# jdalcorso/radar-sounder-crw

Measured on AMD Instinct MI355X. Metric: radargram columns/sec (CRW fwd+bwd), higher is better.
Workload: dtype f32 (conv2-5 multiply on the bf16 matrix cores with hi/lo operand pairs, fp32 accumulate: fp32-grade; everything else fp32); 1 GPU; one synthetic 512x4096 radargram per GPU per step = 8 items [T=32,N=63,16x16] (patch 16x16, overlap (8, 0)), tau=0.01, CNN encoder, fwd+bwd+all-reduce+Adam; parallelism=dp1 (independent sequences), chain=fp32 MFMA 16x16x4, prefix form, encoder_convs=bf16x3

## Files before the change

radar-sounder-crw_amd/csrc/encoder_conv.hip:

```cpp
#include "crw_common.h"
#include <type_traits>
#include <cstdlib>

namespace crw {
namespace {

constexpr int IMG_W = 10, PAD_W = 12, NPIX = 100, NPAD = 144, MT = 7;

typedef __bf16 bf8 __attribute__((ext_vector_type(8)));
typedef short s4v __attribute__((ext_vector_type(4)));
typedef short s8v __attribute__((ext_vector_type(8)));
typedef __attribute__((address_space(3))) char *lds_cp;

__device__ inline uint16_t f2bf(float x) { return __builtin_bit_cast(uint16_t, (__bf16)x); }
__device__ inline float bf2f(uint16_t h) { return __builtin_bit_cast(float, (uint32_t)h << 16); }

template <int C>
constexpr int row_stride() { return C * 2 + 16; }
template <int C>
constexpr int plane_bytes() { return NPAD * row_stride<C>(); }
template <int C>
__device__ inline int px_off(int pp, int chunk) { return pp * row_stride<C>() + 16 * chunk; }
template <int C>
constexpr int crs() { return C * 2 + 32; }
// ... 481 lines not shown
  constexpr int NCO = WG_NCO, NTH = NW * 64;
  constexpr int NPL = (SPLIT == 3) ? 2 : 1;
  constexpr int XS = row_stride<NCI>(), XPL = (XTAIL + NPAD) * XS;
  constexpr int YS = row_stride<NCO>(), YPL = YROWS_ALL * YS;
  constexpr int NT = NCI / 16;
  constexpr int WCI = NT < 4 ? NT : 4, WCO = NW / WCI;
  constexpr int NCOW = NCO / 16 / WCO;
  static_assert(NT == WCI && COUT % NCO == 0 && CIN % NCI == 0, "tiling");
  constexpr int NGRP_CI = CIN / NCI;
  extern __shared__ __attribute__((aligned(16))) char lds[];
  char *xs = lds, *ys = lds + NPL * XPL;

  constexpr int NGRP = NGRP_CI * (COUT / NCO);
  const int wg_slice = a.xcd_map ? ((int)blockIdx.x / 8 / NGRP) * 8 + (int)blockIdx.x % 8 : (int)blockIdx.x / NGRP;
  const int wg_grp = a.xcd_map ? ((int)blockIdx.x / 8) % NGRP : (int)blockIdx.x % NGRP;
  const int grp_ci = wg_grp % NGRP_CI, grp_co = wg_grp / NGRP_CI;
  const int ci_base = grp_ci * NCI, co_base = grp_co * NCO;
  const int tid = threadIdx.x, lane = tid & 63, wave = tid >> 6, g = lane >> 4;
  const int wci = wave % WCI, wco = wave / WCI;
  const int co0w = wco * NCOW * 16;

  f32x4 acc[9][NCOW];
#pragma unroll
  for (int t = 0; t < 9; ++t)
#pragma unroll
    for (int j = 0; j < NCOW; ++j) acc[t][j] = f32x4{0.f, 0.f, 0.f, 0.f};
  f32x4 accb[NCOW];
#pragma unroll
  for (int j = 0; j < NCOW; ++j) accb[j] = f32x4{0.f, 0.f, 0.f, 0.f};
  const bool bias_wave = grp_ci == 0 && __builtin_amdgcn_readfirstlane(wci) == 0;

  const int p_begin = wg_slice * a.patches_per_block;
  const int p_end = min(a.P, p_begin + a.patches_per_block);
  const uint32_t xs_a = (uint32_t)(uintptr_t)(lds_cp)xs, ys_a = (uint32_t)(uintptr_t)(lds_cp)ys;

  for (int pl = 0; pl < NPL; ++pl) {
    zero_halo<NCI, NTH, XS>(xs + pl * XPL + XTAIL * XS, tid);
    for (int c = tid; c < XTAIL * XS / 16; c += NTH) *reinterpret_cast<uint4 *>(xs + pl * XPL + 16 * c) = uint4{0, 0, 0, 0};
    for (int c = tid; c < (1 + TAILPIX) * YS / 16; c += NTH) *reinterpret_cast<uint4 *>(ys + pl * YPL + NPIX * YS + 16 * c) = uint4{0, 0, 0, 0};
  }

  constexpr int XCH = NCI / 8, XTOT = NPIX * XCH, XIT = (XTOT + NTH - 1) / NTH;
  constexpr int YCH = NCO / 8, YTOT = NPIX * YCH, YIT = (YTOT + NTH - 1) / NTH;
  constexpr int TXC = XTAIL * XCH, TYC = TAILPIX * YCH, TTOT = NPL * (TXC + TYC), TIT = (TTOT + NTH - 1) / NTH;
#ifdef CRW_CONV_STAMPS
  long long ph_[4] = {0, 0, 0, 0}, prev_ = (long long)__builtin_amdgcn_s_memtime();
#define WG_STAMP(k) { const long long n_ = (long long)__builtin_amdgcn_s_memtime(); ph_[k] += n_ - prev_; prev_ = n_; }
#else
#define WG_STAMP(k)
#endif

  auto tail_src_dst = [&](int c, int &src, int &dst) {
    const int pl = c / (TXC + TYC), r = c % (TXC + TYC);
    if (r < TXC) {
      const int s = r / XCH, ch = r % XCH;
      dst = pl * XPL + s * XS + 16 * ch;
      src = pl * XPL + (XTAIL + 9 * PAD_W + s) * XS + 16 * ch;
    } else {
      const int q = r - TXC, j = q / YCH, ch = q % YCH;
      dst = NPL * XPL + pl * YPL + (YROWS + j) * YS + 16 * ch;
      src = NPL * XPL + pl * YPL + (NPIX - TAILPIX + j) * YS + 16 * ch;
    }
  };

  const int t16 = lane & 15, q4 = t16 >> 2, pq = t16 & 3;
  const uint32_t lane_col = 8 * (pq & 1) + 16 * (pq >> 1);
  auto row_addr = [&](int v, int carry, bool flush, uint32_t &ya, uint32_t &xa) {
    const int i = v - carry;
    int yrow = NPIX, xpix = XTAIL;
    if (v < carry) {
      const int t = NPIX - carry + v;
      yrow = YROWS + (t - (NPIX - TAILPIX));
      xpix = t - 90;
    } else if (!flush && i < NPIX) {
      yrow = i;
      xpix = XTAIL + (i / IMG_W) * PAD_W + (i % IMG_W);
    }
    ya = ys_a + yrow * YS + lane_col + 2 * co0w;
    xa = xs_a + xpix * XS + lane_col + 32 * wci;
  };
  auto kstep = [&](int ks, int carry, bool flush) {
    uint32_t ya_lo, ya_hi, xa_lo, xa_hi;
    row_addr(32 * ks + 4 * g + q4, carry, flush, ya_lo, xa_lo);
    row_addr(32 * ks + 4 * g + q4 + 16, carry, flush, ya_hi, xa_hi);
    bf8 ah[NCOW], al[NCOW];
    static_for<NCOW>([&](auto JC) {
      constexpr int j = decltype(JC)::value;
      ah[j] = tr_frag<32 * j>(ya_lo, ya_hi);
      if (SPLIT == 3) al[j] = tr_frag<YPL + 32 * j>(ya_lo, ya_hi);
    });
    bf8 bh[2], bl[2];
    auto read_b = [&](auto TC) {
      constexpr int tap = decltype(TC)::value;
      constexpr int XO = ((tap / 3) * PAD_W + (tap % 3)) * XS;
      bh[tap & 1] = tr_frag<XO>(xa_lo, xa_hi);
      if (SPLIT == 3) bl[tap & 1] = tr_frag<XPL + XO>(xa_lo, xa_hi);
    };
    read_b(std::integral_constant<int, 0>{});
    static_for<9>([&](auto TC) {
      constexpr int tap = decltype(TC)::value;
      if constexpr (tap < 8) {
        read_b(std::integral_constant<int, tap + 1>{});
        if (SPLIT == 3) asm volatile("s_waitcnt lgkmcnt(4)" ::: "memory");
        else asm volatile("s_waitcnt lgkmcnt(2)" ::: "memory");
      } else {
        asm volatile("s_waitcnt lgkmcnt(0)" ::: "memory");
      }
      __builtin_amdgcn_sched_barrier(0);
      if constexpr (tap == 0) {
        if (bias_wave) {
          const s8v o = {0x3f80, 0x3f80, 0x3f80, 0x3f80, 0x3f80, 0x3f80, 0x3f80, 0x3f80};
          const bf8 ones = __builtin_bit_cast(bf8, o);
#pragma unroll
          for (int j = 0; j < NCOW; ++j) {
            if (SPLIT == 3) accb[j] = __builtin_amdgcn_mfma_f32_16x16x32_bf16(al[j], ones, accb[j], 0, 0, 0);
            accb[j] = __builtin_amdgcn_mfma_f32_16x16x32_bf16(ah[j], ones, accb[j], 0, 0, 0);
          }
        }
      }
#pragma unroll
      for (int j = 0; j < NCOW; ++j) {
        if (SPLIT == 3) {
          acc[tap][j] = __builtin_amdgcn_mfma_f32_16x16x32_bf16(al[j], bh[tap & 1], acc[tap][j], 0, 0, 0);
          acc[tap][j] = __builtin_amdgcn_mfma_f32_16x16x32_bf16(ah[j], bl[tap & 1], acc[tap][j], 0, 0, 0);
        }
        acc[tap][j] = __builtin_amdgcn_mfma_f32_16x16x32_bf16(ah[j], bh[tap & 1], acc[tap][j], 0, 0, 0);
      }
    });
  };

  int carry = 0;
  uint4 tv[TIT];
#pragma unroll
  for (int i = 0; i < TIT; ++i) tv[i] = uint4{0, 0, 0, 0};
  if constexpr (MAP) {
    const int ntile = a.tiles_x * a.tiles_y;
    constexpr int WTOT = NPAD * XCH, WIT = (WTOT + NTH - 1) / NTH;
    for (int u = p_begin; u < p_end; ++u) {
      const int pq = u / ntile, tile = u % ntile;
      const int ty0 = (tile / a.tiles_x) * IMG_W, tx0 = (tile % a.tiles_x) * IMG_W;
      __syncthreads();
      for (int pl = 0; pl < NPL; ++pl) {
        uint4 xv[WIT];
        const uint16_t *src = (pl ? a.xl : a.xh) + ci_base;
#pragma unroll
        for (int i = 0; i < WIT; ++i) {
          const int c = min(tid + i * NTH, WTOT - 1), wp = c / XCH, ch = c % XCH;
          const int my = ty0 + wp / PAD_W - 1, mx = tx0 + wp % PAD_W - 1;
          const bool ok = my >= 0 && my < a.mh && mx >= 0 && mx < a.mw;
          const long off = (((long)pq * a.mh + min(max(my, 0), a.mh - 1)) * a.mw + min(max(mx, 0), a.mw - 1)) * CIN + 8 * ch;
          xv[i] = *reinterpret_cast<const uint4 *>(src + off);
          if (!ok) xv[i] = uint4{0, 0, 0, 0};
        }
#pragma unroll
        for (int i = 0; i < WIT; ++i) {
          const int c = tid + i * NTH;
          if (WTOT % NTH == 0 || c < WTOT) *reinterpret_cast<uint4 *>(xs + pl * XPL + (XTAIL + c / XCH) * XS + 16 * (c % XCH)) = xv[i];
        }
        uint4 yv[YIT];
        const uint16_t *ysrc = (pl ? a.dyl : a.dyh) + co_base;
#pragma unroll
        for (int i = 0; i < YIT; ++i) {
          const int c = min(tid + i * NTH, YTOT - 1), pix = c / YCH, ch = c % YCH;
          const int oy = ty0 + pix / IMG_W, ox = tx0 + pix % IMG_W;
          const bool ok = oy < a.mh && ox < a.mw;
          const long off = (((long)pq * a.mh + min(oy, a.mh - 1)) * a.mw + min(ox, a.mw - 1)) * COUT + 8 * ch;
          yv[i] = *reinterpret_cast<const uint4 *>(ysrc + off);
          if (!ok) yv[i] = uint4{0, 0, 0, 0};
        }
#pragma unroll
        for (int i = 0; i < YIT; ++i) {
          const int c = tid + i * NTH;
          if (YTOT % NTH == 0 || c < YTOT) *reinterpret_cast<uint4 *>(ys + pl * YPL + (c / YCH) * YS + 16 * (c % YCH)) = yv[i];
        }
      }
      __syncthreads();
#pragma unroll 1
      for (int ks = 0; ks < 4; ++ks) kstep(ks, 0, false);
    }
  }
  for (int p = MAP ? p_end : p_begin; p < p_end; ++p) {
    __syncthreads();
    WG_STAMP(3)
    {
#pragma unroll
      for (int i = 0; i < TIT; ++i) {
        const int c = tid + i * NTH;
        if (TTOT % NTH == 0 || c < TTOT) {
          int src, dst;
          tail_src_dst(c, src, dst);
          *reinterpret_cast<uint4 *>(xs + dst) = tv[i];
        }
      }
      uint4 xv[NPL][XIT], yv[NPL][YIT];
#pragma unroll
      for (int pl = 0; pl < NPL; ++pl) {
        const uint16_t *src = (pl ? a.xl : a.xh) + (long)p * NPIX * CIN + ci_base;
#pragma unroll
        for (int i = 0; i < XIT; ++i) {
          const int c = min(tid + i * NTH, XTOT - 1);
          xv[pl][i] = *reinterpret_cast<const uint4 *>(src + (long)(c / XCH) * CIN + 8 * (c % XCH));
        }
      }
#pragma unroll
      for (int pl = 0; pl < NPL; ++pl) {
        const uint16_t *src = ((pl && !a.dgap) ? a.dyl : a.dyh) + (long)p * NPIX * COUT + co_base;
#pragma unroll
        for (int i = 0; i < YIT; ++i) {
          const int c = min(tid + i * NTH, YTOT - 1);
          yv[pl][i] = *reinterpret_cast<const uint4 *>(src + (long)(c / YCH) * COUT + 8 * (c % YCH));
        }
      }
#pragma unroll
      for (int pl = 0; pl < NPL; ++pl)
#pragma unroll
        for (int i = 0; i < XIT; ++i) {
          const int c = tid + i * NTH;
          if (XTOT % NTH == 0 || c < XTOT)
            *reinterpret_cast<uint4 *>(xs + pl * XPL + (XTAIL + interior_pp(c / XCH)) * XS + 16 * (c % XCH)) = xv[pl][i];
        }
      if (a.dgap) {
        static_assert(NTH % YCH == 0, "a thread keeps its channel chunk");
        const int ch = tid % YCH;
        uint32_t gh[4], gl[4];
        gap_split8(a.dgap + (long)p * COUT + co_base + 8 * ch, gh, gl);
#pragma unroll
        for (int i = 0; i < YIT; ++i) {
          const int c = tid + i * NTH;
          if (YTOT % NTH == 0 || c < YTOT) {
            uint4 oh, ol;
            gap_mask8(yv[0][i], gh, gl, oh, ol);
            const int off = (c / YCH) * YS + 16 * ch;
            *reinterpret_cast<uint4 *>(ys + off) = oh;
            if (SPLIT == 3) *reinterpret_cast<uint4 *>(ys + YPL + off) = ol;
          }
        }
      } else {
#pragma unroll
        for (int pl = 0; pl < NPL; ++pl)
#pragma unroll
          for (int i = 0; i < YIT; ++i) {
            const int c = tid + i * NTH;
            if (YTOT % NTH == 0 || c < YTOT) *reinterpret_cast<uint4 *>(ys + pl * YPL + (c / YCH) * YS + 16 * (c % YCH)) = yv[pl][i];
          }
      }
    }
    __syncthreads();
    WG_STAMP(0)
    WG_STAMP(1)
#ifdef CRW_CONV_STAMPS
    if (a.stamps && tid == 0 && p - p_begin < 60)
      a.stamps[(long)blockIdx.x * 64 + 4 + (p - p_begin)] = (long long)__builtin_amdgcn_s_memtime();
#endif
    const int nks = carry == 8 ? 4 : 3;
#pragma unroll 1
    for (int ks = 0; ks < nks; ++ks) kstep(ks, carry, false);
    carry = carry == 8 ? 0 : carry + 4;
#pragma unroll
    for (int i = 0; i < TIT; ++i) {
      const int c = min(tid + i * NTH, TTOT - 1);
      int src, dst;
      tail_src_dst(c, src, dst);
      tv[i] = *reinterpret_cast<const uint4 *>(xs + src);
    }
    WG_STAMP(2)
  }
  if (carry > 0) {
    __syncthreads();
#pragma unroll
    for (int i = 0; i < TIT; ++i) {
      const int c = tid + i * NTH;
      if (TTOT % NTH == 0 || c < TTOT) {
        int src, dst;
        tail_src_dst(c, src, dst);
        *reinterpret_cast<uint4 *>(xs + dst) = tv[i];
      }
    }
    __syncthreads();
    kstep(0, carry, true);
  }
#ifdef CRW_CONV_STAMPS
  if (a.stamps && tid == 0)
    for (int k = 0; k < 4; ++k) a.stamps[(long)blockIdx.x * 64 + k] = ph_[k];
#endif

  float *dwp = a.dw_part + (long)wg_slice * COUT * CIN * 9;
#pragma unroll
  for (int tap = 0; tap < 9; ++tap)
#pragma unroll
    for (int j = 0; j < NCOW; ++j)
#pragma unroll
      for (int r = 0; r < 4; ++r) {
        const int co = co_base + co0w + 16 * j + 4 * g + r, ci = ci_base + 16 * wci + (lane & 15);
        dwp[((long)tap * COUT + co) * CIN + ci] = acc[tap][j][r];
      }
  if (bias_wave && (lane & 15) == 0) {
#pragma unroll
    for (int j = 0; j < NCOW; ++j)
#pragma unroll
      for (int r = 0; r < 4; ++r) a.db_part[(long)wg_slice * COUT + co_base + co0w + 16 * j + 4 * g + r] = accb[j][r];
  }
}

constexpr int W2_NCO = 128, W2_NCI = 64, W2_NW = 8, W2_KROWS = 32;
template <int C>
constexpr int w2_stride() { return 2 * C + 32; }

template <int SPLIT, int CIN, int COUT, int DIAG = 0>
__global__ __launch_bounds__(W2_NW * 64, 2) void conv3x3_wgrad2_kernel(WgradArgs a) {
  constexpr int NCO = W2_NCO, NCI = W2_NCI, NTH = W2_NW * 64, NPL = (SPLIT == 3) ? 2 : 1;
  constexpr int XS = w2_stride<NCI>(), XPL = NPAD * XS, XSLOT = NPL * XPL;
  constexpr int YS = w2_stride<NCO>(), YPL = W2_KROWS * YS, YSLOT = NPL * YPL;
  constexpr int NCOW = 4, WCI = 4;
  static_assert(COUT == NCO && CIN % NCI == 0, "tiling");
  constexpr int NGRP = CIN / NCI;
  extern __shared__ __attribute__((aligned(16))) char lds[];
  char *xs = lds, *ys = lds + 2 * XSLOT;
  char *gs = ys + 2 * YSLOT;

  const int wg_slice = a.xcd_map ? ((int)blockIdx.x / 8 / NGRP) * 8 + (int)blockIdx.x % 8 : (int)blockIdx.x / NGRP;
  const int grp_ci = a.xcd_map ? ((int)blockIdx.x / 8) % NGRP : (int)blockIdx.x % NGRP;
  const int ci_base = grp_ci * NCI;
  const int tid = threadIdx.x, lane = tid & 63, wave = tid >> 6, g = lane >> 4;
  const int wci = wave % WCI, wco = wave / WCI;
  const int wci_s = __builtin_amdgcn_readfirstlane(wci);
  const int co0w = wco * NCOW * 16;

  const int p_begin = wg_slice * a.patches_per_block;
  const int np = min(a.P, p_begin + a.patches_per_block) - p_begin;
  const int npx = np * NPIX;
  const int NK = (npx + W2_KROWS - 1) / W2_KROWS;

  f32x4 acc[9][NCOW];
#pragma unroll
  for (int t = 0; t < 9; ++t)
#pragma unroll
    for (int j = 0; j < NCOW; ++j) acc[t][j] = f32x4{0.f, 0.f, 0.f, 0.f};
  f32x4 accb = f32x4{0.f, 0.f, 0.f, 0.f};
  const bool bias_wg = grp_ci == 0;

  for (int c = tid; c < 2 * XSLOT / 16; c += NTH) *reinterpret_cast<uint4 *>(xs + 16 * c) = uint4{0, 0, 0, 0};

  const int yrow = tid >> 4, ych = tid & 15;
  constexpr int XCH = NCI / 8, XTOT = NPIX * XCH;
  typedef uint32_t u4v __attribute__((ext_vector_type(4)));
  const long dy_off = (long)p_begin * NPIX * COUT, x_off = (long)p_begin * NPIX * CIN + ci_base;
  const __amdgpu_buffer_rsrc_t dyh_rs = __builtin_amdgcn_make_buffer_rsrc((void *)(a.dyh + dy_off), 0, npx * COUT * 2, 0x00020000);
  const __amdgpu_buffer_rsrc_t dyl_rs = __builtin_amdgcn_make_buffer_rsrc(
      (void *)((SPLIT == 3 && !a.dgap ? a.dyl : a.dyh) + dy_off), 0, npx * COUT * 2, 0x00020000);
  const __amdgpu_buffer_rsrc_t xh_rs = __builtin_amdgcn_make_buffer_rsrc((void *)(a.xh + x_off), 0, (npx * CIN - ci_base) * 2, 0x00020000);
  const __amdgpu_buffer_rsrc_t xl_rs = __builtin_amdgcn_make_buffer_rsrc((void *)((SPLIT == 3 ? a.xl : a.xh) + x_off), 0,
                                                                          (npx * CIN - ci_base) * 2, 0x00020000);
  const int y_voff = (yrow * COUT + 8 * ych) * 2;
  int x_voff[2];
#pragma unroll
  for (int i = 0; i < 2; ++i) {
    const int c = min(tid + i * NTH, XTOT - 1);
    x_voff[i] = ((c / XCH) * CIN + 8 * (c % XCH)) * 2;
  }
  uint4 sy[NPL], sx[2];
  auto load_dy = [&](int n) {
    const int soff = n * (W2_KROWS * COUT * 2);
    constexpr int AUX = DIAG == 6 ? 2 : 0;
    sy[0] = __builtin_bit_cast(uint4, (u4v)__builtin_amdgcn_raw_buffer_load_b128(dyh_rs, y_voff, soff, AUX));
    if (SPLIT == 3 && !a.dgap) sy[NPL - 1] = __builtin_bit_cast(uint4, (u4v)__builtin_amdgcn_raw_buffer_load_b128(dyl_rs, y_voff, soff, AUX));
  };
  auto store_dy = [&](int n) {
    uint4 vh = sy[0], vl = uint4{0, 0, 0, 0};
    if (SPLIT == 3 && !a.dgap) vl = sy[NPL - 1];
    if (a.dgap) {
      const int q = (32 * n + yrow) / NPIX;
      const uint4 h4 = *reinterpret_cast<const uint4 *>(gs + (q & 1) * (4 * COUT) + 16 * ych);
      const uint4 l4 = *reinterpret_cast<const uint4 *>(gs + (q & 1) * (4 * COUT) + 2 * COUT + 16 * ych);
      const uint32_t gh[4] = {h4.x, h4.y, h4.z, h4.w}, gl[4] = {l4.x, l4.y, l4.z, l4.w};
      gap_mask8(sy[0], gh, gl, vh, vl);
    }
    char *dst = ys + (n & 1) * YSLOT + yrow * YS + 16 * ych;
    *reinterpret_cast<uint4 *>(dst) = vh;
    if (SPLIT == 3) *reinterpret_cast<uint4 *>(dst + YPL) = vl;
  };
  auto load_x = [&](int q, int pl) {
    const int soff = q * (NPIX * CIN * 2);
#pragma unroll
    for (int i = 0; i < 2; ++i)
      sx[i] = __builtin_bit_cast(uint4, (u4v)__builtin_amdgcn_raw_buffer_load_b128(pl ? xl_rs : xh_rs, x_voff[i], soff, DIAG == 6 ? 2 : 0));
  };
  auto store_x = [&](int q, int pl) {
    char *dst = xs + (q & 1) * XSLOT + pl * XPL;
#pragma unroll
    for (int i = 0; i < 2; ++i) {
      const int c = tid + i * NTH;
      if (c < XTOT) *reinterpret_cast<uint4 *>(dst + interior_pp(c / XCH) * XS + 16 * (c % XCH)) = sx[i];
    }
  };
  auto stage_gap = [&](int q) {
    if (tid < COUT / 8) {
      uint32_t gh[4], gl[4];
      gap_split8(a.dgap + (long)(p_begin + q) * COUT + 8 * tid, gh, gl);
      *reinterpret_cast<uint4 *>(gs + (q & 1) * (4 * COUT) + 16 * tid) = uint4{gh[0], gh[1], gh[2], gh[3]};
      *reinterpret_cast<uint4 *>(gs + (q & 1) * (4 * COUT) + 2 * COUT + 16 * tid) = uint4{gl[0], gl[1], gl[2], gl[3]};
    }
  };
  auto first_k = [&](int q) { return (q * NPIX) / W2_KROWS; };
  auto patch_starting_at = [&](int n) {
    if (n >= NK) return -1;
    const int q = min((32 * n + 31) / NPIX, np - 1);
    return first_k(q) == n ? q : -1;
  };

  const uint32_t xs_a = (uint32_t)(uintptr_t)(lds_cp)xs, ys_a = (uint32_t)(uintptr_t)(lds_cp)ys;
  const int t16 = lane & 15, q4 = t16 >> 2, pq = t16 & 3;
  const uint32_t lane_col = 8 * (pq & 1) + 16 * (pq >> 1);
  const int r_lo = 4 * g + q4, r_hi = r_lo + 16;
  const uint32_t ya_lo0 = ys_a + r_lo * YS + lane_col + 2 * co0w, ya_hi0 = ys_a + r_hi * YS + lane_col + 2 * co0w;
  auto x_addr = [&](int G) {
    const int Gc = min(G, npx - 1);
    const int q = Gc / NPIX, i = Gc - q * NPIX;
    return xs_a + (q & 1) * XSLOT + ((i / IMG_W) * PAD_W + (i % IMG_W)) * XS + lane_col + 32 * wci;
  };

  auto kstep = [&](int n) {
    const uint32_t ya_lo = ya_lo0 + (n & 1) * YSLOT, ya_hi = ya_hi0 + (n & 1) * YSLOT;
    const uint32_t xa_lo = x_addr(32 * n + r_lo), xa_hi = x_addr(32 * n + r_hi);
    bf8 ah[NCOW], al[NCOW];
    static_for<NCOW>([&](auto JC) {
      constexpr int j = decltype(JC)::value;
      ah[j] = tr_frag<32 * j>(ya_lo, ya_hi);
      if (SPLIT == 3) al[j] = tr_frag<YPL + 32 * j>(ya_lo, ya_hi);
    });
    bf8 bh[2], bl[2];
    auto read_b = [&](auto TC) {
      constexpr int tap = decltype(TC)::value;
      constexpr int XO = ((tap / 3) * PAD_W + (tap % 3)) * XS;
      bh[tap & 1] = tr_frag<XO>(xa_lo, xa_hi);
      if (SPLIT == 3) bl[tap & 1] = tr_frag<XPL + XO>(xa_lo, xa_hi);
    };
    read_b(std::integral_constant<int, 0>{});
    static_for<9>([&](auto TC) {
      constexpr int tap = decltype(TC)::value;
      if constexpr (tap < 8) {
        read_b(std::integral_constant<int, tap + 1>{});
        if (SPLIT == 3) asm volatile("s_waitcnt lgkmcnt(4)" ::: "memory");
        else asm volatile("s_waitcnt lgkmcnt(2)" ::: "memory");
      } else {
        asm volatile("s_waitcnt lgkmcnt(0)" ::: "memory");
      }
      __builtin_amdgcn_sched_barrier(0);
      if constexpr (tap == 0) {
        if (bias_wg) {
          const s8v o = {0x3f80, 0x3f80, 0x3f80, 0x3f80, 0x3f80, 0x3f80, 0x3f80, 0x3f80};
          const bf8 ones = __builtin_bit_cast(bf8, o);
          static_for<NCOW>([&](auto JC) {
            constexpr int j = decltype(JC)::value;
            if (wci_s == j) {
              if (SPLIT == 3) accb = __builtin_amdgcn_mfma_f32_16x16x32_bf16(al[j], ones, accb, 0, 0, 0);
              accb = __builtin_amdgcn_mfma_f32_16x16x32_bf16(ah[j], ones, accb, 0, 0, 0);
            }
          });
        }
      }
#pragma unroll
      for (int j = 0; j < NCOW; ++j) {
        if (SPLIT == 3) {
          acc[tap][j] = __builtin_amdgcn_mfma_f32_16x16x32_bf16(al[j], bh[tap & 1], acc[tap][j], 0, 0, 0);
          acc[tap][j] = __builtin_amdgcn_mfma_f32_16x16x32_bf16(ah[j], bl[tap & 1], acc[tap][j], 0, 0, 0);
        }
        acc[tap][j] = __builtin_amdgcn_mfma_f32_16x16x32_bf16(ah[j], bh[tap & 1], acc[tap][j], 0, 0, 0);
      }
    });
  };

  load_dy(0);
  load_x(0, 0);
  if (a.dgap) stage_gap(0);
  __syncthreads();
  store_x(0, 0);
  if (SPLIT == 3) {
    load_x(0, 1);
    store_x(0, 1);
  }
  store_dy(0);
  __syncthreads();

#pragma unroll 1
  for (int n = 0; n < NK; ++n) {
    const bool more = n + 1 < NK;
    const int q_2 = patch_starting_at(n + 2);
    const int q_hi = (SPLIT == 3) ? q_2 : -1;
    const int q_lo = patch_starting_at(n + 1);
    const int xq = q_lo >= 0 ? q_lo : q_hi, xpl = q_lo >= 0 ? NPL - 1 : 0;
    if (DIAG != 2 && DIAG != 3 && DIAG != 5) {
      load_dy(more ? n + 1 : n);
      load_x(xq >= 0 ? xq : 0, xpl);
    }
    kstep(n);
    if (DIAG == 2 || DIAG == 3) {
      if (DIAG & 1) continue;
      __syncthreads();
      continue;
    }
    if (DIAG == 4) {
      asm volatile("" ::"v"(sy[0].x), "v"(sy[NPL - 1].y), "v"(sx[0].x), "v"(sx[1].y));
      __syncthreads();
      continue;
    }
    if (more) store_dy(n + 1);
    if (xq >= 0) store_x(xq, xpl);
    if (a.dgap && q_2 >= 0) stage_gap(q_2);
    if (!(DIAG & 1)) __syncthreads();
  }

  float *dwp = a.dw_part + (long)wg_slice * COUT * CIN * 9;
#pragma unroll
  for (int tap = 0; tap < 9; ++tap)
#pragma unroll
    for (int j = 0; j < NCOW; ++j)
#pragma unroll
      for (int r = 0; r < 4; ++r) {
        const int co = co0w + 16 * j + 4 * g + r, ci = ci_base + 16 * wci + (lane & 15);
        dwp[((long)tap * COUT + co) * CIN + ci] = acc[tap][j][r];
      }
  if (bias_wg && (lane & 15) == 0) {
#pragma unroll
    for (int r = 0; r < 4; ++r) a.db_part[(long)wg_slice * COUT + co0w + 16 * wci + 4 * g + r] = accb[r];
  }
}

__global__ __launch_bounds__(256) void slice_sum_kernel(const float *__restrict__ part, int nslice, long n,
                                                        float *__restrict__ out) {
  for (long e = (long)blockIdx.x * 256 + threadIdx.x; e < n; e += (long)gridDim.x * 256) {
    float s = 0.f;
    for (int k = 0; k < nslice; ++k) s += part[(long)k * n + e];
    out[e] = s;
  }
}

__global__ __launch_bounds__(256) void slice_sum_dw_kernel(const float *__restrict__ part, int nslice, int coci,
                                                           float *__restrict__ out, int nblk_dw,
                                                           const float *__restrict__ bpart, int cout, float *__restrict__ bout) {
  __shared__ float red[4][64];
  const long n = 9L * coci;
  const int lane = threadIdx.x & 63, q = threadIdx.x >> 6;
  if ((int)blockIdx.x >= nblk_dw) {
    const int e = ((int)blockIdx.x - nblk_dw) * 4 + q;
    if (e >= cout) return;
    float s = 0.f;
    for (int k = lane; k < nslice; k += 64) s += bpart[(long)k * cout + e];
    s = wave_sum(s);
    if (lane == 0) bout[e] = s;
    return;
  }
  const long e = (long)blockIdx.x * 64 + lane;
  const int per = (nslice + 3) / 4, k0 = q * per, k1 = min(nslice, k0 + per);
  float s = 0.f;
  if (e < n) {
    int k = k0;
    for (; k + 8 <= k1; k += 8) {
      float v[8];
#pragma unroll
      for (int u = 0; u < 8; ++u) v[u] = part[(long)(k + u) * n + e];
#pragma unroll
      for (int u = 0; u < 8; ++u) s += v[u];
    }
    for (; k < k1; ++k) s += part[(long)k * n + e];
  }
  red[q][lane] = s;
  __syncthreads();
  if (q == 0 && e < n) {
    const float t = (red[0][lane] + red[1][lane]) + (red[2][lane] + red[3][lane]);
    const int tap = e / coci, cc = e % coci;
    out[(long)cc * 9 + tap] = t;
  }
}

__device__ inline long frag_index(int tap, int n, int k, int N, int K) {
  return ((((long)tap * (K / 32) + k / 32) * (N / 16) + n / 16) * 64 + ((k % 32) / 8) * 16 + n % 16) * 8 + k % 8;
}
__global__ __launch_bounds__(256) void pack_weights_kernel(const float *__restrict__ w, int CO, int CI,
                                                           uint16_t *fh, uint16_t *fl, uint16_t *bh, uint16_t *bl) {
  const long n = (long)CO * CI * 9;
  for (long e = (long)blockIdx.x * 256 + threadIdx.x; e < n; e += (long)gridDim.x * 256) {
    const int tap = e % 9, ci = (e / 9) % CI, co = e / (9L * CI);
    const float v = w[e];
    const uint16_t h = f2bf(v), l = f2bf(v - bf2f(h));
    const long of = frag_index(tap, co, ci, CO, CI), ob = frag_index(8 - tap, ci, co, CI, CO);
    fh[of] = h; bh[ob] = h;
    if (fl) { fl[of] = l; bl[ob] = l; }
  }
}

__global__ __launch_bounds__(256) void pack_input_kernel(const float *__restrict__ x, int P, int C, int npix, uint16_t *xh,
                                                         uint16_t *xl) {
  const long n = (long)P * npix * C;
  for (long e = (long)blockIdx.x * 256 + threadIdx.x; e < n; e += (long)gridDim.x * 256) {
    const int c = e % C, i = (e / C) % npix;
    const long p = e / ((long)C * npix);
    const float v = x[(p * C + c) * npix + i];
    const uint16_t h = f2bf(v);
    xh[e] = h;
    if (xl) xl[e] = f2bf(v - bf2f(h));
  }
}

__global__ __launch_bounds__(256) void gap_bwd_kernel(const float *__restrict__ dgap, const uint16_t *__restrict__ yh,
                                                      int P, int C, int npix, uint16_t *dh, uint16_t *dl) {
  const long n8 = (long)P * npix * C / 8;
  const int c8 = C / 8;
  const float inv = 1.0f / (float)npix;
  for (long e = (long)blockIdx.x * 256 + threadIdx.x; e < n8; e += (long)gridDim.x * 256) {
#pragma clang fp contract(off)
    const int c = (int)(e % c8) * 8;
    const long p = e / ((long)c8 * npix);
    const uint4 y = *reinterpret_cast<const uint4 *>(yh + e * 8);
    const float4 g0 = *reinterpret_cast<const float4 *>(dgap + p * C + c), g1 = *reinterpret_cast<const float4 *>(dgap + p * C + c + 4);
    const float gv[8] = {g0.x, g0.y, g0.z, g0.w, g1.x, g1.y, g1.z, g1.w};
    const uint32_t yw[4] = {y.x, y.y, y.z, y.w};
    uint32_t h[4], l[4];
#pragma unroll
    for (int w = 0; w < 4; ++w) {
      const float a0 = (yw[w] & 0x7fffu) ? gv[2 * w] * inv : 0.f, a1 = (yw[w] & 0x7fff0000u) ? gv[2 * w + 1] * inv : 0.f;
      const uint16_t h0 = f2bf(a0), h1 = f2bf(a1);
      h[w] = (uint32_t)h0 | ((uint32_t)h1 << 16);
      l[w] = (uint32_t)f2bf(a0 - bf2f(h0)) | ((uint32_t)f2bf(a1 - bf2f(h1)) << 16);
    }
    *reinterpret_cast<uint4 *>(dh + e * 8) = uint4{h[0], h[1], h[2], h[3]};
    if (dl) *reinterpret_cast<uint4 *>(dl + e * 8) = uint4{l[0], l[1], l[2], l[3]};
  }
}

template <int C>
constexpr size_t conv_lds_bytes(int npl) { return (size_t)(npl - 1) * PLANE_ROWS * crs<C>() + (size_t)NPAD * crs<C>(); }

template <int SPLIT, int CIN, int COUT, int MODE, int NW>
int launch_conv_nw(const ConvArgs &a, hipStream_t s) {
  constexpr int CMAX = CIN > COUT ? CIN : COUT;
  size_t lds = conv_lds_bytes<CMAX>(SPLIT == 3 ? 2 : 1);
#ifdef CRW_CONV_STAMPS
  if (const char *e = getenv("CRW_CONV_LDS_PAD")) lds += (size_t)atoi(e);
#endif
  static bool attr = false;
  if (!attr && lds > 64 * 1024) {
    if (hipFuncSetAttribute((const void *)conv3x3_kernel<SPLIT, CIN, COUT, MODE, NW>,
                            hipFuncAttributeMaxDynamicSharedMemorySize, (int)lds) != hipSuccess) {
      g_last_hip_error = (int)hipGetLastError();
      return CRW_EHIP;
    }
    attr = true;
  }
  hipLaunchKernelGGL((conv3x3_kernel<SPLIT, CIN, COUT, MODE, NW>), dim3(a.P), dim3(NW * 64), lds, s, a);
  return check_launch();
}

constexpr int MT_SMALL = 4;

template <int SPLIT, int CIN, int COUT, int MODE, int MTL>
int launch_conv_map_cls(const ConvArgs &a, hipStream_t s) {
  constexpr int CMAX = CIN > COUT ? CIN : COUT, NW = (SPLIT == 3 ? 8 : 4);
  const size_t lds = (size_t)(SPLIT == 3 ? 2 : 1) * NPAD * row_stride<CMAX>();
  static bool attr = false;
  if (!attr && lds > 64 * 1024) {
    if (hipFuncSetAttribute((const void *)conv3x3_kernel<SPLIT, CIN, COUT, MODE, NW, true, MTL>,
                            hipFuncAttributeMaxDynamicSharedMemorySize, (int)lds) != hipSuccess) {
      g_last_hip_error = (int)hipGetLastError();
      return CRW_EHIP;
    }
    attr = true;
  }
  hipLaunchKernelGGL((conv3x3_kernel<SPLIT, CIN, COUT, MODE, NW, true, MTL>), dim3(a.P * a.ncls), dim3(NW * 64), lds, s, a);
  return check_launch();
}

template <int SPLIT, int CIN, int COUT, int MODE = 0>
int launch_conv_map(const ConvArgs &a0, hipStream_t s) {
  const int ntile = a0.tiles_x * a0.tiles_y;
  if (ntile > 65535) return CRW_EINVAL;
  constexpr int CHUNK = (int)(sizeof(a0.tile_list) / sizeof(a0.tile_list[0]));
  ConvArgs big = a0, small = a0;
  big.ncls = small.ncls = 0;
  for (int t = 0; t < ntile; ++t) {
    const int th = std::min(IMG_W, a0.mh - (t / a0.tiles_x) * IMG_W), tw = std::min(IMG_W, a0.mw - (t % a0.tiles_x) * IMG_W);
    if (tw * th > 16 * MT_SMALL) {
      big.tile_list[big.ncls++] = (unsigned short)t;
      if (big.ncls == CHUNK) {
        CRW_TRY((launch_conv_map_cls<SPLIT, CIN, COUT, MODE, MT>(big, s)));
        big.ncls = 0;
      }
    } else {
      small.tile_list[small.ncls++] = (unsigned short)t;
      if (small.ncls == CHUNK) {
        CRW_TRY((launch_conv_map_cls<SPLIT, CIN, COUT, MODE, MT_SMALL>(small, s)));
        small.ncls = 0;
      }
    }
  }
  if (big.ncls) CRW_TRY((launch_conv_map_cls<SPLIT, CIN, COUT, MODE, MT>(big, s)));
  if (small.ncls) CRW_TRY((launch_conv_map_cls<SPLIT, CIN, COUT, MODE, MT_SMALL>(small, s)));
  return CRW_OK;
}

template <int SPLIT, int CIN, int COUT, int MODE>
int launch_conv(const ConvArgs &a, hipStream_t s) {
  static const char *force = getenv("CRW_CONV_NW");
  if (force && force[0] == '4') return launch_conv_nw<SPLIT, CIN, COUT, MODE, 4>(a, s);
  if (force && force[0] == '8') return launch_conv_nw<SPLIT, CIN, COUT, MODE, 8>(a, s);
  return launch_conv_nw<SPLIT, CIN, COUT, MODE, (SPLIT == 3 ? 8 : 4)>(a, s);
}

constexpr int wgrad_nci(int cin) { return cin > 64 ? 64 : cin; }

template <int SPLIT, int CIN, int COUT>
int launch_wgrad(const WgradArgs &a, int nblk, hipStream_t s) {
  constexpr int NCI = wgrad_nci(CIN), NW = SPLIT == 3 ? 4 : 8;
  const size_t lds = (size_t)(SPLIT == 3 ? 2 : 1) * ((XTAIL + NPAD) * row_stride<NCI>() + YROWS_ALL * row_stride<WG_NCO>());
  static bool attr = false;
  if (!attr && lds > 64 * 1024) {
    if (hipFuncSetAttribute((const void *)conv3x3_wgrad_kernel<SPLIT, CIN, COUT, NCI, NW>,
                            hipFuncAttributeMaxDynamicSharedMemorySize, (int)lds) != hipSuccess) {
      g_last_hip_error = (int)hipGetLastError();
      return CRW_EHIP;
    }
    attr = true;
  }
  hipLaunchKernelGGL((conv3x3_wgrad_kernel<SPLIT, CIN, COUT, NCI, NW>), dim3(nblk * (CIN / NCI) * (COUT / WG_NCO)),
                     dim3(NW * 64), lds, s, a);
  return check_launch();
}

template <int SPLIT, int CIN, int COUT>
int launch_wgrad_map(const WgradArgs &a, int nblk, hipStream_t s) {
  constexpr int NCI = wgrad_nci(CIN), NW = SPLIT == 3 ? 4 : 8;
  const size_t lds = (size_t)(SPLIT == 3 ? 2 : 1) * ((XTAIL + NPAD) * row_stride<NCI>() + YROWS_ALL * row_stride<WG_NCO>());
  static bool attr = false;
  if (!attr && lds > 64 * 1024) {
    if (hipFuncSetAttribute((const void *)conv3x3_wgrad_kernel<SPLIT, CIN, COUT, NCI, NW, true>,
                            hipFuncAttributeMaxDynamicSharedMemorySize, (int)lds) != hipSuccess) {
      g_last_hip_error = (int)hipGetLastError();
      return CRW_EHIP;
    }
    attr = true;
  }
  hipLaunchKernelGGL((conv3x3_wgrad_kernel<SPLIT, CIN, COUT, NCI, NW, true>), dim3(nblk * (CIN / NCI) * (COUT / WG_NCO)),
                     dim3(NW * 64), lds, s, a);
  return check_launch();
}

template <int SPLIT, int CIN, int COUT, int DIAG = 0>
int launch_wgrad2(const WgradArgs &a, int nslice, hipStream_t s) {
  constexpr int NPL = SPLIT == 3 ? 2 : 1;
  const size_t lds = (size_t)2 * NPL * (NPAD * w2_stride<W2_NCI>() + W2_KROWS * w2_stride<W2_NCO>()) + 2 * 4 * W2_NCO;
  static bool attr = false;
  if (!attr) {
    if (hipFuncSetAttribute((const void *)conv3x3_wgrad2_kernel<SPLIT, CIN, COUT, DIAG>, hipFuncAttributeMaxDynamicSharedMemorySize,
                            (int)lds) != hipSuccess) {
      g_last_hip_error = (int)hipGetLastError();
      return CRW_EHIP;
    }
    attr = true;
  }
  hipLaunchKernelGGL((conv3x3_wgrad2_kernel<SPLIT, CIN, COUT, DIAG>), dim3(nslice * (CIN / W2_NCI)), dim3(W2_NW * 64), lds, s, a);
  return check_launch();
}

inline int ew_grid(long n) {
  long b = (n + 255) / 256;
  return (int)(b > 8192 ? 8192 : (b < 1 ? 1 : b));
}

}
}

using namespace crw;

long long *g_conv_stamps = nullptr;

extern "C" {

#ifdef CRW_CONV_STAMPS
void crw_debug_conv_stamps(long long *buf) { g_conv_stamps = buf; }
#endif

int crw_enc_pack_weights(const float *w, int cout, int cin, uint16_t *fwd_hi, uint16_t *fwd_lo, uint16_t *bwd_hi,
                         uint16_t *bwd_lo, crw_stream_t stream) {
  clear_stale_error();
  if (!w || !fwd_hi || !bwd_hi || cout < 1 || cin < 1 || (fwd_lo == nullptr) != (bwd_lo == nullptr)) return CRW_EINVAL;
  hipLaunchKernelGGL(pack_weights_kernel, dim3(ew_grid((long)cout * cin * 9)), dim3(256), 0, (hipStream_t)stream, w, cout,
                     cin, fwd_hi, fwd_lo, bwd_hi, bwd_lo);
  return check_launch();
}

int crw_enc_pack_input(const float *x, int P, int C, uint16_t *xh, uint16_t *xl, crw_stream_t stream) {
  clear_stale_error();
  if (!x || !xh || P < 1 || C < 8 || C % 8) return CRW_EINVAL;
  hipLaunchKernelGGL(pack_input_kernel, dim3(ew_grid((long)P * NPIX * C)), dim3(256), 0, (hipStream_t)stream, x, P, C,
                     NPIX, xh, xl);
  return check_launch();
}

int crw_enc_pack_input_map(const float *x, int P, int C, int H, int W, uint16_t *xh, uint16_t *xl, crw_stream_t stream) {
  clear_stale_error();
  if (!x || !xh || P < 1 || C < 8 || C % 8 || H < 1 || W < 1) return CRW_EINVAL;
  hipLaunchKernelGGL(pack_input_kernel, dim3(ew_grid((long)P * H * W * C)), dim3(256), 0, (hipStream_t)stream, x, P, C,
                     H * W, xh, xl);
  return check_launch();
}

int crw_enc_conv3x3_map(int mode, int split, int P, int H, int W, int cin, int cout, const uint16_t *x_hi, const uint16_t *x_lo,
                        const uint16_t *w_hi, const uint16_t *w_lo, const float *bias, const uint16_t *mask_hi, uint16_t *y_hi,
                        uint16_t *y_lo, float *y_f32, float *gap_part, crw_stream_t stream) {
  clear_stale_error();
  if (!x_hi || !w_hi || P < 1 || H < 1 || W < 1 || (split != 1 && split != 3) || (mode != 0 && mode != 1)) return CRW_EINVAL;
  if (split == 3 && (!w_lo || !x_lo)) return CRW_EINVAL;
  if (!y_hi && !gap_part && !y_f32) return CRW_EINVAL;
  if (mode == 1 && (gap_part || bias)) return CRW_EINVAL;
  const int tx = (W + IMG_W - 1) / IMG_W, ty = (H + IMG_W - 1) / IMG_W;
  if ((long)P * tx * ty > 0x7fffffffL) return CRW_EINVAL;
  ConvArgs a{x_hi, x_lo, w_hi, w_lo, bias, mask_hi, y_hi, y_lo, y_f32, gap_part, nullptr, P, nullptr, H, W, tx, ty, 0, {}};
  hipStream_t s = (hipStream_t)stream;
#define CRW_MAP_CASE(CI, CO, MODE) \
  if (mode == MODE && cin == CI && cout == CO) return split == 3 ? launch_conv_map<3, CI, CO, MODE>(a, s) : launch_conv_map<1, CI, CO, MODE>(a, s);
  CRW_MAP_CASE(32, 64, 0)
  CRW_MAP_CASE(64, 128, 0)
  CRW_MAP_CASE(128, 128, 0)
  CRW_MAP_CASE(128, 128, 1)
  CRW_MAP_CASE(128, 64, 1)
  CRW_MAP_CASE(64, 32, 1)
#undef CRW_MAP_CASE
  return CRW_EINVAL;
}

int crw_enc_gap_bwd(const float *dgap, const uint16_t *y_hi, int P, int C, int npix, uint16_t *dy_hi, uint16_t *dy_lo,
                    crw_stream_t stream) {
  clear_stale_error();
  if (!dgap || !y_hi || !dy_hi || P < 1 || C < 8 || C % 8 || npix < 1) return CRW_EINVAL;
  hipLaunchKernelGGL(gap_bwd_kernel, dim3(ew_grid((long)P * npix * C / 8)), dim3(256), 0, (hipStream_t)stream, dgap, y_hi, P,
                     C, npix, dy_hi, dy_lo);
  return check_launch();
}

int crw_enc_conv3x3(int mode, int split, int P, int cin, int cout, const uint16_t *x_hi, const uint16_t *x_lo,
                    const uint16_t *w_hi, const uint16_t *w_lo, const float *bias, const uint16_t *mask_hi,
                    uint16_t *y_hi, uint16_t *y_lo, float *y_f32, float *gap, const float *dgap, crw_stream_t stream) {
  clear_stale_error();
  if (!x_hi || !w_hi || P < 1 || (mode != 0 && mode != 1) || (split != 1 && split != 3)) return CRW_EINVAL;
  if (split == 3 && (!w_lo || (!x_lo && !dgap))) return CRW_EINVAL;
  if (dgap && mode != 1) return CRW_EINVAL;
  if (!y_hi && !y_f32 && !gap) return CRW_EINVAL;
  ConvArgs a{x_hi, x_lo, w_hi, w_lo, bias, mask_hi, y_hi, y_lo, y_f32, gap, dgap, P, g_conv_stamps, 0, 0, 1, 1};
  hipStream_t s = (hipStream_t)stream;
#define CRW_CONV_CASE(CI, CO)                                                                      \
  if (cin == CI && cout == CO) {                                                                   \
    if (split == 3) return mode == 0 ? launch_conv<3, CI, CO, 0>(a, s) : launch_conv<3, CI, CO, 1>(a, s); \
    return mode == 0 ? launch_conv<1, CI, CO, 0>(a, s) : launch_conv<1, CI, CO, 1>(a, s);           \
  }
  CRW_CONV_CASE(32, 64)
  CRW_CONV_CASE(64, 128)
  CRW_CONV_CASE(128, 128)
  CRW_CONV_CASE(128, 64)
  CRW_CONV_CASE(64, 32)
#undef CRW_CONV_CASE
  return CRW_EINVAL;
}

static int wgrad_groups(int cin) { return cin / wgrad_nci(cin); }

static int wgrad_slices(int P, int cin, int cout, int split) {
  (void)split;
  const int groups = wgrad_groups(cin) * (cout / WG_NCO);
  int n = 256 * 2 / (groups < 1 ? 1 : groups);
  return n > P ? P : n;
}

size_t crw_enc_wgrad_ws_bytes(int P, int cin, int cout, int split) {
  if (P < 1 || cin < 1 || cout < 1) return 0;
  return (size_t)wgrad_slices(P, cin, cout, split) *
         ((size_t)cout * cin * 9 + (size_t)wgrad_groups(cin) * cout) * sizeof(float);
}

int crw_enc_conv3x3_wgrad(int split, int P, int cin, int cout, const uint16_t *dy_hi, const uint16_t *dy_lo,
                          const uint16_t *x_hi, const uint16_t *x_lo, const float *dgap, float *dw, float *db, void *ws,
                          size_t ws_bytes, crw_stream_t stream) {
  clear_stale_error();
  if (!dy_hi || !x_hi || !dw || !db || !ws || P < 1 || (split != 1 && split != 3)) return CRW_EINVAL;
  if (split == 3 && ((!dy_lo && !dgap) || !x_lo)) return CRW_EINVAL;
  if (ws_bytes < crw_enc_wgrad_ws_bytes(P, cin, cout, split)) return CRW_EWORKSPACE;
  hipStream_t s = (hipStream_t)stream;
  int nslice = wgrad_slices(P, cin, cout, split);
  static const char *force = getenv("CRW_WGRAD");
  const bool streamed = cout == W2_NCO && cin % W2_NCI == 0 && !(force && force[0] == '1');
  if (streamed) {
    const int n2 = 256 / (cin / W2_NCI);
    nslice = n2 > P ? P : n2;
  }
  int ppb = (P + nslice - 1) / nslice;
  if (streamed) nslice = (P + ppb - 1) / ppb;
  float *dw_part = static_cast<float *>(ws), *db_part = dw_part + (size_t)nslice * cout * cin * 9;
  WgradArgs a{dy_hi, dy_lo, x_hi, x_lo, dgap, dw_part, db_part, P, ppb, nslice % 8 == 0 ? 1 : 0, g_conv_stamps, 0, 0, 1, 1};
  int st = CRW_EINVAL;
  if (streamed) {
    if (cin == 64) st = split == 3 ? launch_wgrad2<3, 64, 128>(a, nslice, s) : launch_wgrad2<1, 64, 128>(a, nslice, s);
    else if (cin == 128) {
#ifdef CRW_CONV_STAMPS
      static const char *diag = getenv("CRW_WGRAD_DIAG");
      if (diag && split == 3 && diag[0] == '1') return launch_wgrad2<3, 128, 128, 1>(a, nslice, s);
      if (diag && split == 3 && diag[0] == '2') return launch_wgrad2<3, 128, 128, 2>(a, nslice, s);
      if (diag && split == 3 && diag[0] == '3') return launch_wgrad2<3, 128, 128, 3>(a, nslice, s);
      if (diag && split == 3 && diag[0] == '4') return launch_wgrad2<3, 128, 128, 4>(a, nslice, s);
      if (diag && split == 3 && diag[0] == '5') return launch_wgrad2<3, 128, 128, 5>(a, nslice, s);
      if (diag && split == 3 && diag[0] == '6') return launch_wgrad2<3, 128, 128, 6>(a, nslice, s);
#endif
      st = split == 3 ? launch_wgrad2<3, 128, 128>(a, nslice, s) : launch_wgrad2<1, 128, 128>(a, nslice, s);
    }
  } else {
#define CRW_WG_CASE(CI, CO)                                                                  \
  if (cin == CI && cout == CO) st = split == 3 ? launch_wgrad<3, CI, CO>(a, nslice, s) : launch_wgrad<1, CI, CO>(a, nslice, s);
  CRW_WG_CASE(32, 64)
  CRW_WG_CASE(64, 128)
  CRW_WG_CASE(128, 128)
#undef CRW_WG_CASE
  }
  if (st != CRW_OK) return st;
  const long nw = (long)cout * cin * 9;
  const int nblk_dw = (int)((nw + 63) / 64);
  hipLaunchKernelGGL(slice_sum_dw_kernel, dim3((unsigned)(nblk_dw + (cout + 3) / 4)), dim3(256), 0, s, dw_part, nslice, cout * cin,
                     dw, nblk_dw, db_part, cout, db);
  return check_launch();
}


int crw_enc_conv3x3_wgrad_map(int split, int P, int H, int W, int cin, int cout, const uint16_t *dy_hi, const uint16_t *dy_lo,
                              const uint16_t *x_hi, const uint16_t *x_lo, float *dw, float *db, void *ws, size_t ws_bytes,
                              crw_stream_t stream) {
  clear_stale_error();
  if (!dy_hi || !x_hi || !dw || !db || !ws || P < 1 || H < 1 || W < 1 || (split != 1 && split != 3)) return CRW_EINVAL;
  if (split == 3 && (!dy_lo || !x_lo)) return CRW_EINVAL;
  const int tx = (W + IMG_W - 1) / IMG_W, ty = (H + IMG_W - 1) / IMG_W;
  const long units_l = (long)P * tx * ty;
  if (units_l > 0x7fffffffL) return CRW_EINVAL;
  const int units = (int)units_l;
  if (ws_bytes < crw_enc_wgrad_ws_bytes(units, cin, cout, split)) return CRW_EWORKSPACE;
  hipStream_t s = (hipStream_t)stream;
  int nslice = wgrad_slices(units, cin, cout, split);
  const int upb = (units + nslice - 1) / nslice;
  nslice = (units + upb - 1) / upb;
  float *dw_part = static_cast<float *>(ws), *db_part = dw_part + (size_t)nslice * cout * cin * 9;
  WgradArgs a{dy_hi, dy_lo, x_hi, x_lo, nullptr, dw_part, db_part, units, upb, nslice % 8 == 0 ? 1 : 0, nullptr, H, W, tx, ty};
  int st = CRW_EINVAL;
#define CRW_WGM_CASE(CI, CO) \
  if (cin == CI && cout == CO) st = split == 3 ? launch_wgrad_map<3, CI, CO>(a, nslice, s) : launch_wgrad_map<1, CI, CO>(a, nslice, s);
  CRW_WGM_CASE(32, 64)
  CRW_WGM_CASE(64, 128)
  CRW_WGM_CASE(128, 128)
#undef CRW_WGM_CASE
  if (st != CRW_OK) return st;
  const long nw = (long)cout * cin * 9;
  const int nblk_dw = (int)((nw + 63) / 64);
  hipLaunchKernelGGL(slice_sum_dw_kernel, dim3((unsigned)(nblk_dw + (cout + 3) / 4)), dim3(256), 0, s, dw_part, nslice, cout * cin,
                     dw, nblk_dw, db_part, cout, db);
  return check_launch();
}

}
```

Before: 651,800 radargram columns/s.

## Route conv3 weight gradient through streamed wgrad2 kernel with generalized tiling

Generalizes the streamed weight-gradient kernel so the wave count, channel tile and LDS size derive from CIN/COUT, letting the 32->64 conv3 layer use it instead of the older per-slice kernel. Conv3 gets 512 slices to keep the GPU filled with the smaller 256-thread workgroups. It also points idle X prefetches at a zero-size buffer resource so out-of-range loads return nothing rather than re-fetching patch 0. The trade-off is more partial-sum slices to reduce and a new tiling path that is only checked by static asserts.

Measured after the change: 663,900 radargram columns/s, median of 6. No clear change (+1.9%).

```diff
diff --git a/radar-sounder-crw_amd/csrc/encoder_conv.hip b/radar-sounder-crw_amd/csrc/encoder_conv.hip
--- a/radar-sounder-crw_amd/csrc/encoder_conv.hip
+++ b/radar-sounder-crw_amd/csrc/encoder_conv.hip
@@ -807,17 +807,23 @@
   }
 }
 
-constexpr int W2_NCO = 128, W2_NCI = 64, W2_NW = 8, W2_KROWS = 32;
+constexpr int W2_NCO = 128, W2_NCI = 64, W2_KROWS = 32;
+constexpr int w2_nci(int cin) { return cin < W2_NCI ? cin : W2_NCI; }
+constexpr int w2_nw(int cin, int cout) { return cout / (w2_nci(cin) / 16) / 16 * (w2_nci(cin) / 16); }
 template <int C>
 constexpr int w2_stride() { return 2 * C + 32; }
+template <int SPLIT, int CIN, int COUT>
+constexpr size_t w2_lds_bytes() {
+  return (size_t)2 * (SPLIT == 3 ? 2 : 1) * (NPAD * w2_stride<w2_nci(CIN)>() + W2_KROWS * w2_stride<COUT>()) + 2 * 4 * COUT;
+}
 
 template <int SPLIT, int CIN, int COUT, int DIAG = 0>
-__global__ __launch_bounds__(W2_NW * 64, 2) void conv3x3_wgrad2_kernel(WgradArgs a) {
-  constexpr int NCO = W2_NCO, NCI = W2_NCI, NTH = W2_NW * 64, NPL = (SPLIT == 3) ? 2 : 1;
+__global__ __launch_bounds__(w2_nw(CIN, COUT) * 64, 2) void conv3x3_wgrad2_kernel(WgradArgs a) {
+  constexpr int NCO = COUT, NCI = w2_nci(CIN), NTH = w2_nw(CIN, COUT) * 64, NPL = (SPLIT == 3) ? 2 : 1;
   constexpr int XS = w2_stride<NCI>(), XPL = NPAD * XS, XSLOT = NPL * XPL;
   constexpr int YS = w2_stride<NCO>(), YPL = W2_KROWS * YS, YSLOT = NPL * YPL;
-  constexpr int NCOW = 4, WCI = 4;
-  static_assert(COUT == NCO && CIN % NCI == 0, "tiling");
+  constexpr int WCI = NCI / 16, NCOW = WCI;
+  static_assert(CIN % NCI == 0 && NCI % 16 == 0 && NTH == (NCO / (16 * NCOW)) * WCI * 64 && NCO == 2 * NCOW * 16, "tiling");
   constexpr int NGRP = CIN / NCI;
   extern __shared__ __attribute__((aligned(16))) char lds[];
   char *xs = lds, *ys = lds + 2 * XSLOT;
@@ -846,8 +852,11 @@
 
   for (int c = tid; c < 2 * XSLOT / 16; c += NTH) *reinterpret_cast<uint4 *>(xs + 16 * c) = uint4{0, 0, 0, 0};
 
-  const int yrow = tid >> 4, ych = tid & 15;
+  constexpr int YCH = NCO / 8;
+  static_assert(W2_KROWS * YCH == NTH, "one dY chunk per thread");
+  const int yrow = tid / YCH, ych = tid % YCH;
   constexpr int XCH = NCI / 8, XTOT = NPIX * XCH;
+  static_assert(XTOT <= 2 * NTH, "two X chunks per thread");
   typedef uint32_t u4v __attribute__((ext_vector_type(4)));
   const long dy_off = (long)p_begin * NPIX * COUT, x_off = (long)p_begin * NPIX * CIN + ci_base;
   const __amdgpu_buffer_rsrc_t dyh_rs = __builtin_amdgcn_make_buffer_rsrc((void *)(a.dyh + dy_off), 0, npx * COUT * 2, 0x00020000);
@@ -856,6 +865,7 @@
   const __amdgpu_buffer_rsrc_t xh_rs = __builtin_amdgcn_make_buffer_rsrc((void *)(a.xh + x_off), 0, (npx * CIN - ci_base) * 2, 0x00020000);
   const __amdgpu_buffer_rsrc_t xl_rs = __builtin_amdgcn_make_buffer_rsrc((void *)((SPLIT == 3 ? a.xl : a.xh) + x_off), 0,
                                                                           (npx * CIN - ci_base) * 2, 0x00020000);
+  const __amdgpu_buffer_rsrc_t x0_rs = __builtin_amdgcn_make_buffer_rsrc((void *)(a.xh + x_off), 0, 0, 0x00020000);
   const int y_voff = (yrow * COUT + 8 * ych) * 2;
   int x_voff[2];
 #pragma unroll
@@ -885,10 +895,15 @@
     if (SPLIT == 3) *reinterpret_cast<uint4 *>(dst + YPL) = vl;
   };
   auto load_x = [&](int q, int pl) {
-    const int soff = q * (NPIX * CIN * 2);
+    const int soff = (q >= 0 ? q : 0) * (NPIX * CIN * 2);
+#ifdef CRW_W2_IDLE_X
+    const __amdgpu_buffer_rsrc_t rs = pl ? xl_rs : xh_rs;
+#else
+    const __amdgpu_buffer_rsrc_t rs = q < 0 ? x0_rs : pl ? xl_rs : xh_rs;
+#endif
 #pragma unroll
     for (int i = 0; i < 2; ++i)
-      sx[i] = __builtin_bit_cast(uint4, (u4v)__builtin_amdgcn_raw_buffer_load_b128(pl ? xl_rs : xh_rs, x_voff[i], soff, DIAG == 6 ? 2 : 0));
+      sx[i] = __builtin_bit_cast(uint4, (u4v)__builtin_amdgcn_raw_buffer_load_b128(rs, x_voff[i], soff, DIAG == 6 ? 2 : 0));
   };
   auto store_x = [&](int q, int pl) {
     char *dst = xs + (q & 1) * XSLOT + pl * XPL;
@@ -996,7 +1011,7 @@
     const int xq = q_lo >= 0 ? q_lo : q_hi, xpl = q_lo >= 0 ? NPL - 1 : 0;
     if (DIAG != 2 && DIAG != 3 && DIAG != 5) {
       load_dy(more ? n + 1 : n);
-      load_x(xq >= 0 ? xq : 0, xpl);
+      load_x(xq, xpl);
     }
     kstep(n);
     if (DIAG == 2 || DIAG == 3) {
@@ -1251,8 +1266,7 @@
 
 template <int SPLIT, int CIN, int COUT, int DIAG = 0>
 int launch_wgrad2(const WgradArgs &a, int nslice, hipStream_t s) {
-  constexpr int NPL = SPLIT == 3 ? 2 : 1;
-  const size_t lds = (size_t)2 * NPL * (NPAD * w2_stride<W2_NCI>() + W2_KROWS * w2_stride<W2_NCO>()) + 2 * 4 * W2_NCO;
+  const size_t lds = w2_lds_bytes<SPLIT, CIN, COUT>();
   static bool attr = false;
   if (!attr) {
     if (hipFuncSetAttribute((const void *)conv3x3_wgrad2_kernel<SPLIT, CIN, COUT, DIAG>, hipFuncAttributeMaxDynamicSharedMemorySize,
@@ -1262,7 +1276,8 @@
     }
     attr = true;
   }
-  hipLaunchKernelGGL((conv3x3_wgrad2_kernel<SPLIT, CIN, COUT, DIAG>), dim3(nslice * (CIN / W2_NCI)), dim3(W2_NW * 64), lds, s, a);
+  hipLaunchKernelGGL((conv3x3_wgrad2_kernel<SPLIT, CIN, COUT, DIAG>), dim3(nslice * (CIN / w2_nci(CIN))),
+                     dim3(w2_nw(CIN, COUT) * 64), lds, s, a);
   return check_launch();
 }
 
@@ -1391,9 +1406,10 @@
   hipStream_t s = (hipStream_t)stream;
   int nslice = wgrad_slices(P, cin, cout, split);
   static const char *force = getenv("CRW_WGRAD");
-  const bool streamed = cout == W2_NCO && cin % W2_NCI == 0 && !(force && force[0] == '1');
+  const bool conv3 = cin == 32 && cout == 64;
+  const bool streamed = ((cout == W2_NCO && cin % W2_NCI == 0) || conv3) && !(force && force[0] == '1');
   if (streamed) {
-    const int n2 = 256 / (cin / W2_NCI);
+    const int n2 = conv3 ? 2 * 256 : 256 / (cin / W2_NCI);
     nslice = n2 > P ? P : n2;
   }
   int ppb = (P + nslice - 1) / nslice;
@@ -1402,7 +1418,8 @@
   WgradArgs a{dy_hi, dy_lo, x_hi, x_lo, dgap, dw_part, db_part, P, ppb, nslice % 8 == 0 ? 1 : 0, g_conv_stamps, 0, 0, 1, 1};
   int st = CRW_EINVAL;
   if (streamed) {
-    if (cin == 64) st = split == 3 ? launch_wgrad2<3, 64, 128>(a, nslice, s) : launch_wgrad2<1, 64, 128>(a, nslice, s);
+    if (conv3) st = split == 3 ? launch_wgrad2<3, 32, 64>(a, nslice, s) : launch_wgrad2<1, 32, 64>(a, nslice, s);
+    else if (cin == 64) st = split == 3 ? launch_wgrad2<3, 64, 128>(a, nslice, s) : launch_wgrad2<1, 64, 128>(a, nslice, s);
     else if (cin == 128) {
 #ifdef CRW_CONV_STAMPS
       static const char *diag = getenv("CRW_WGRAD_DIAG");
```
